# CornellHPC/HySortK

Hardware: AMD Instinct MI355X
Metric: k-mers counted/sec at K=31 (higher is better)
Workload: dtype u64

## Files before the change

hysortk_amd/csrc/hsk_parse.h:

```cpp
#pragma once
#include "hsk_device.h"

namespace hsk {

constexpr int PARSE_THREADS = 256;
constexpr int PARSE_PPT = 8;
constexpr int PARSE_TILE = PARSE_THREADS * PARSE_PPT;
constexpr int SUPERMER_CUT = 128;
constexpr int MAX_K = 95;
constexpr int HSK_MAX_TASKS = 1024;
constexpr int PARSE_WORDS = PARSE_TILE / 16 + 12;
constexpr int PARSE_HMAX = PARSE_TILE + 96;
constexpr int PARSE_RWIN = 64;
static_assert(PARSE_RWIN + PARSE_WORDS <= PARSE_THREADS, "scan_kernel prefetches the next tile with one lane per read-index entry and per word");

struct BinTable { u32 *cursor; u32 *map; u32 vmax; u32 cap_chunks; u32 *ctl; u32 *chunk_bin; ulonglong2 *items; u32 *subs; u32 *err; };

struct ParseArgs {
    const u8 *packed;
    u64 packed_bytes;
    const u64 *roff;
    const u32 *rlen;
    u64 nreads;
    int k, m;
// ... 567 lines not shown
            }
        }
        lds_barrier();
        if (a.packed_copy && tid < PARSE_TILE / 16 && bbase + 4u * (u64)tid < a.packed_bytes)
            a.packed_copy[(bbase >> 2) + tid] = __builtin_bswap32(s_words[tid]);
        {
            const u64 nb = bbase + PARSE_TILE / 4;
            pf_have = (ti + 1 < a.tiles_per_block) && (tile + 1 < tile_end) && (nb + (u64)PARSE_WORDS * 4 <= a.packed_bytes);
            if (pf_have) {
                if (tid < PARSE_RWIN) {
                    const u64 idx = s_rng[1] + tid;
                    const u64 o_ = (idx <= a.nreads) ? a.roff[idx] : RINF;
                    pf0 = (u32)o_; pf1 = (u32)(o_ >> 32);
                    pf2 = (idx < a.nreads) ? a.rlen[idx] : 0;
                } else if (tid < PARSE_RWIN + PARSE_WORDS) pf0 = reinterpret_cast<const u32 *>(a.packed + nb)[tid - PARSE_RWIN];
            }
        }
#ifdef HSK_DIAG
        if (tid == 0) { unsigned long long t_ = __builtin_amdgcn_s_memtime(); sd[1] = t_; }
#endif

        u64 h[PARSE_PPT];
        {
            const u64 w0 = bits64_be32(s_words, 16u * (u32)tid);
            const u64 rw = ~rev2(w0);
#pragma unroll
            for (int i = 0; i < PARSE_PPT; ++i) {
                const u64 fw = (w0 << (2 * i)) & mmask;
                const u64 rc = (rw << (2 * (32 - M - i))) & mmask;
                h[i] = murmur64_8(rc < fw ? rc : fw);
            }
#pragma unroll
            for (int i = 0; i < PARSE_PPT; ++i) s_hash[i * SCAN_HSTRIDE + tid] = h[i];
            if (W >= 2 * PARSE_PPT) {
                u64 bm = h[0];
#pragma unroll
                for (int i = 1; i < PARSE_PPT; ++i) bm = h[i] < bm ? h[i] : bm;
                s_bmin[tid] = bm;
            }
            for (int e = PARSE_THREADS - 1 - tid; e < W - 1; e += PARSE_THREADS) {
                const int p = PARSE_TILE + e;
                const u64 fw = bits64_be32(s_words, 2u * (u32)p) & mmask;
                const u64 tw = twin1(fw, M);
                s_hash[scan_hidx(p)] = murmur64_8(tw < fw ? tw : fw);
            }
        }
        lds_barrier();
#ifdef HSK_DIAG
        if (tid == 0) { unsigned long long t_ = __builtin_amdgcn_s_memtime(); sd[2] = t_; }
#endif

        u64 mn[PARSE_PPT];
        if (W >= PARSE_PPT) {
            u64 c = h[PARSE_PPT - 1];
            const int nfull = (W - PARSE_PPT) / PARSE_PPT;
            int j = PARSE_PPT;
            if (nfull > 0 && tid + nfull < PARSE_THREADS) {
                for (int b = 1; b <= nfull; ++b) { const u64 v = s_bmin[tid + b]; c = v < c ? v : c; }
                j = PARSE_PPT * (nfull + 1);
            }
#pragma unroll 8
            for (; j <= W - 1; ++j) { const u64 v = s_hash[scan_hidx(p0 + j)]; c = v < c ? v : c; }
            mn[PARSE_PPT - 1] = c;
            u64 suf = ~0ULL;
#pragma unroll
            for (int i = PARSE_PPT - 2; i >= 0; --i) { suf = h[i] < suf ? h[i] : suf; mn[i] = suf < c ? suf : c; }
            u64 run = ~0ULL;
#pragma unroll
            for (int i = 1; i < PARSE_PPT; ++i) { const u64 v = s_hash[scan_hidx(p0 + W + i - 1)]; run = v < run ? v : run; mn[i] = run < mn[i] ? run : mn[i]; }
        } else {
#pragma unroll
            for (int i = 0; i < PARSE_PPT; ++i) {
                u64 c = ~0ULL;
                for (int j = 0; j < W; ++j) { const u64 v = s_hash[scan_hidx(p0 + i + j)]; c = v < c ? v : c; }
                mn[i] = c;
            }
        }
        u32 vmask = 0;
        {
            const u64 g0 = gbase + p0;
            const u64 rlo = s_rng[0], rhi = s_rng[1], rb = s_rng[2];
            const bool fast = s_rng[3] != 0;
            u64 r, rstart, rend, nxt;
            if (fast) {
                u32 lo = (u32)(rlo - rb), hi = (u32)(rhi - rb);
                const u64 b0 = g0 >> 2;
                while (lo < hi) { const u32 mid = (lo + hi + 1) >> 1; if (s_roff[mid] <= b0) lo = mid; else hi = mid - 1; }
                r = rb + lo; rstart = s_roff[lo] * 4; rend = rstart + s_rlen[lo];
                nxt = (r + 1 < a.nreads) ? s_roff[lo + 1] * 4 : ~0ULL;
            } else {
                r = find_read(a.roff, rlo, rhi, g0 >> 2);
                rstart = a.roff[r] * 4; rend = rstart + a.rlen[r];
                nxt = (r + 1 < a.nreads) ? a.roff[r + 1] * 4 : ~0ULL;
            }
            if (nxt >= g0 + PARSE_PPT) {
                const long long cnt = (long long)rend - (long long)K - (long long)g0 + 1;
                vmask = cnt <= 0 ? 0u : (cnt >= PARSE_PPT ? 0xFFu : ((1u << (u32)cnt) - 1u));
            } else {
                static_assert(PARSE_PPT == 8, "two bytes of bases per lane");
                const long long cnt_lo = (long long)rend - (long long)K - (long long)g0 + 1;
                vmask = cnt_lo <= 0 ? 0u : (cnt_lo >= 4 ? 0xFu : ((1u << (u32)cnt_lo) - 1u));
                do {
                    ++r; rstart = nxt;
                    if (fast) { const u32 j = (u32)(r - rb); rend = rstart + s_rlen[j]; nxt = (r + 1 < a.nreads) ? s_roff[j + 1] * 4 : ~0ULL; }
                    else { rend = rstart + a.rlen[r]; nxt = (r + 1 < a.nreads) ? a.roff[r + 1] * 4 : ~0ULL; }
                } while (nxt <= g0 + 4);
                const long long cnt_hi = (long long)rend - (long long)K - (long long)(g0 + 4) + 1;
                vmask |= (cnt_hi <= 0 ? 0u : (cnt_hi >= 4 ? 0xFu : ((1u << (u32)cnt_hi) - 1u))) << 4;
            }
        }
        if constexpr (DROP) {
            const u32 dm = homopolymer_positions(s_words, tid, K, a.drop_mask);
            ndrop += (u32)__popc(vmask & dm);
            vmask &= ~dm;
        }
        s_last[tid] = mn[PARSE_PPT - 1];
        s_v8[tid] = (u8)vmask;
        lds_barrier();
#ifdef HSK_DIAG
        if (tid == 0) { unsigned long long t_ = __builtin_amdgcn_s_memtime(); sd[3] = t_; }
#endif

        u32 start8 = 0;
        {
            u64 pm = tid ? s_last[tid - 1] : 0;
            const u32 pv = tid ? (u32)(s_v8[tid - 1] >> 7) : 0u;
            u32 neq8 = 0;
#pragma unroll
            for (int i = 0; i < PARSE_PPT; ++i) { neq8 |= (mn[i] != pm ? 1u : 0u) << i; pm = mn[i]; }
            const u32 cut8 = ((tid & (SUPERMER_CUT / PARSE_PPT - 1)) == 0) ? 1u : 0u;
            const u32 prev8 = (vmask << 1) | pv;
            const u32 bnd8 = (~vmask | cut8 | ~prev8 | neq8) & 0xFFu;
            s_bnd8[tid] = (u8)bnd8;
            if (tid == 0) s_scan[10] = 0;
            start8 = vmask & bnd8;
        }
        u32 nrec;
        u32 off = block_excl_scan_256_lds<u32>((u32)__popc(start8), s_scan, &nrec);
#pragma unroll
        for (int i = 0; i < PARSE_PPT; ++i)
            if ((start8 >> i) & 1) { s_hash[off] = mn[i]; s_plist[off] = (u16)(p0 + i); ++off; }
        lds_barrier();
#ifdef HSK_DIAG
        if (tid == 0) { unsigned long long t_ = __builtin_amdgcn_s_memtime(); sd[4] = t_; }
#endif

        if (BINS) complete_pending(s_wprev);
        {
            const u64 *bw = reinterpret_cast<const u64 *>(s_bnd8);
            u32 *trec = a.tile_rec + tile * (u64)a.rec_cap;
            for (u32 r = tid; r < nrec; r += PARSE_THREADS) {
                const u32 p = s_plist[r];
                u32 d = fastmod64(s_hash[r], a.fm);
                const u32 sub = (u32)((s_hash[r] * 0x9E3779B97F4A7C15ULL) >> 32);
                if (a.vt_shift) d = (d << a.vt_shift) | (sub >> (32u - a.vt_shift));
                const u32 w = p >> 6;
                const u64 m = ((p & 63) == 63) ? 0ULL : (bw[w] & (~0ULL << ((p & 63) + 1)));
                u32 nb = (p | (SUPERMER_CUT - 1)) + 1;
                if (m) nb = w * 64 + (u32)__builtin_ctzll(m);
                else if ((w & 1) == 0) { const u64 m2 = bw[w + 1]; if (m2) nb = (w + 1) * 64 + (u32)__builtin_ctzll(m2); }
                u32 nk = nb - p;
                if constexpr (BINS) {
                    const BinTable &bt = *a.bins;
                    const u32 bin = xcc_nvt + d;
                    for (u32 pp = p, rest = nk, first = 1u; rest; first = 0u) {
                        const u32 piece = rest < maxk ? rest : maxk;
                        atomicAdd((unsigned long long *)&s_cur[2 * d + 0], (1ULL << 40) | (unsigned long long)piece);
                        const u32 pos = bin_reserve(bt, bin);
                        if (first && r < 2u * PARSE_THREADS) {
                            s_pend[r] = make_uint2(pp | (piece << 11) | (d << 16), sub);
                            if (r < (u32)PARSE_THREADS) { pend_pos0 = pos; pend_mask |= 1u; } else { pend_pos1 = pos; pend_mask |= 2u; }
                        } else bin_store(bt, bin_slot(bt, bin, pos, s_mc, d), bits64_be32(s_words, 2u * pp), bits64_be32(s_words, 2u * pp + 64u), piece, sub);
                        pp += piece; rest -= piece;
                    }
                    continue;
                }
                if (a.tile_sub && nk > maxk) {
                    for (u32 pp = p + maxk, rest = nk - maxk; rest; ) {
                        const u32 piece = rest < maxk ? rest : maxk;
                        const u32 rx = nrec + atomicAdd(&s_scan[10], 1u);
                        atomicAdd((unsigned long long *)&s_cur[2 * d + 0], (1ULL << 40) | (unsigned long long)piece);
                        atomicAdd((unsigned long long *)&s_cur[2 * d + 1], (unsigned long long)((piece + K - 1 + 3) >> 2));
                        if (rx < a.rec_cap) { trec[rx] = pp | ((piece - 1) << 11) | (d << 18); a.tile_sub[tile * (u64)a.rec_cap + rx] = sub; }
                        pp += piece; rest -= piece;
                    }
                    nk = maxk;
                }
                atomicAdd((unsigned long long *)&s_cur[2 * d + 0], (1ULL << 40) | (unsigned long long)nk);
                atomicAdd((unsigned long long *)&s_cur[2 * d + 1], (unsigned long long)((nk + K - 1 + 3) >> 2));
                if (r < a.rec_cap) { trec[r] = p | ((nk - 1) << 11) | (d << 18); if (a.tile_sub) a.tile_sub[tile * (u64)a.rec_cap + r] = sub; }
            }
        }
        lds_barrier();
        if (tid == 0 && !BINS) {
            const u32 nall = nrec + s_scan[10];
            a.tile_nrec[tile] = nall;
            if (nall > a.rec_cap) atomicOr(a.overflow, 1u);
        }
#ifdef HSK_DIAG
        if (tid == 0) { unsigned long long t_ = __builtin_amdgcn_s_memtime(); sd[5] = t_; }
#endif
#ifdef HSK_DIAG
        if (tid == 0) { for (int q = 0; q < 5; ++q) dacc[q] += sd[q + 1] - sd[q]; dacc[5] += 1; }
#endif
    }
#ifdef HSK_DIAG
    if (tid == 0) { for (int q = 0; q < 5; ++q) atomicAdd(&g_scan_diag[q], dacc[q]); atomicAdd(&g_scan_diag[8], dacc[5]); }
#endif
    if (BINS) complete_pending(s_words2[BINS ? (wsel ^ 1u) : 0u]);
    if constexpr (DROP) {
        u32 v = ndrop;
        for (int o = 32; o > 0; o >>= 1) v += __shfl_down(v, o, WAVE);
        if (lane_id() == 0 && v) atomicAdd(a.dropped, (unsigned long long)v);
    }
    for (u32 t = tid; t < a.ntasks; t += PARSE_THREADS) {
        u64 *o = a.blk_cnt + ((u64)blockIdx.x * a.ntasks + t) * 3;
        const u64 pk = s_cur[2 * t];
        const u64 bytes_t = BINS ? 0ULL : s_cur[2 * t + 1];
        if (a.slab == 0 || a.place_one) { o[0] = pk >> 40; o[1] = bytes_t; o[2] = pk & ((1ULL << 40) - 1); }
        else { o[0] += pk >> 40; o[1] += bytes_t; o[2] += pk & ((1ULL << 40) - 1); }
    }
}

__global__ __launch_bounds__(PARSE_THREADS) void place_kernel(ParseArgs a)
{
    if (a.place_one && a.overflow && *(const volatile u32 *)a.overflow) return;
    constexpr int RPT = PLACE_MAX_REC / PARSE_THREADS;
    __shared__ u32 s_scan[12];
    __shared__ u32 s_go[20];
    extern __shared__ __attribute__((aligned(16))) u64 s_cur[];
    const int tid = threadIdx.x;
    const int K = a.k;
    u32 *s_tcnt = reinterpret_cast<u32 *>(s_cur + a.ntasks);
    u32 *s_tpre = s_tcnt + a.ntasks;
    u32 *s_srt = s_tpre + a.ntasks;
    for (u32 t = tid; t < a.ntasks; t += PARSE_THREADS) s_cur[t] = a.blk_base[((u64)blockIdx.x * a.ntasks + t) * 2];
    const u32 G = a.place_group;
    const u32 nsl = a.nslabs > 1 ? a.nslabs : 1;
    for (u32 sl = a.place_one ? a.slab : 0; sl < (a.place_one ? a.slab + 1 : nsl); ++sl) {
    const u64 tile0 = (u64)sl * a.slab_tiles + (u64)blockIdx.x * a.tiles_per_block;
    const u64 tile_end = (nsl > 1 && ((u64)sl + 1) * a.slab_tiles < a.ntiles) ? ((u64)sl + 1) * a.slab_tiles : a.ntiles;
    for (u32 t0 = 0; t0 < a.tiles_per_block; t0 += G) {
        const u64 tfirst = tile0 + t0;
        if (tfirst >= tile_end) break;
        u32 ng = a.tiles_per_block - t0; if (ng > G) ng = G;
        if (tfirst + ng > tile_end) ng = (u32)(tile_end - tfirst);
        __syncthreads();
        if (tid == 0) {
            u32 run = 0;
            for (u32 j = 0; j < ng; ++j) { s_go[j] = run; u32 n = a.tile_nrec[tfirst + j]; run += n < a.rec_cap ? n : a.rec_cap; }
            for (u32 j = ng; j <= 16; ++j) s_go[j] = run;
        }
        for (u32 t = tid; t < a.ntasks; t += PARSE_THREADS) s_tcnt[t] = 0;
        __syncthreads();
        const u32 total = s_go[16];
        u32 rec[RPT], rnk[RPT];
#pragma unroll
        for (int x = 0; x < RPT; ++x) {
            const u32 i = x * PARSE_THREADS + tid;
            rec[x] = 0xFFFFFFFFu;
            if (i < total) {
                u32 j = 0;
                while (j + 1 < ng && s_go[j + 1] <= i) ++j;
                const u32 r = a.tile_rec[(tfirst + j) * (u64)a.rec_cap + (i - s_go[j])];
                rec[x] = r | (j << 28);
                rnk[x] = atomicAdd(&s_tcnt[(r >> 18) & 1023u], 1u);
            }
        }
        __syncthreads();
        {
            u32 c4[4], sum = 0;
#pragma unroll
            for (int j = 0; j < 4; ++j) { const u32 t = tid * 4 + j; c4[j] = t < a.ntasks ? s_tcnt[t] : 0; sum += c4[j]; }
            u32 e = block_excl_scan_256<u32>(sum, s_scan, nullptr);
#pragma unroll
            for (int j = 0; j < 4; ++j) { const u32 t = tid * 4 + j; if (t < a.ntasks) s_tpre[t] = e; e += c4[j]; }
        }
        __syncthreads();
#pragma unroll
        for (int x = 0; x < RPT; ++x)
            if (rec[x] != 0xFFFFFFFFu) s_srt[s_tpre[(rec[x] >> 18) & 1023u] + rnk[x]] = rec[x];
        __syncthreads();
        for (u32 i = tid; i < total; i += PARSE_THREADS) {
            const u32 r = s_srt[i];
            const u32 d = (r >> 18) & 1023u;
            if (a.task_skip && a.task_skip[d]) continue;
            const u64 slot = s_cur[d] + (i - s_tpre[d]);
            a.sm_len[slot] = (u8)(((r >> 11) & 127) + K);
            a.sm_gpos[slot] = (tfirst + (r >> 28)) * PARSE_TILE + (u64)(r & 2047);
        }
        __syncthreads();
        for (u32 t = tid; t < a.ntasks; t += PARSE_THREADS) s_cur[t] += s_tcnt[t];
    }
    }
}

constexpr int PLACE_ITEM_THREADS = 1024;
#ifndef PLACE_ITEM_RPT
#define PLACE_ITEM_RPT 16
#endif
constexpr u32 PLACE_ITEM_REC = PLACE_ITEM_RPT * 1024;
constexpr u32 PLACE_ITEM_TILES = PLACE_ITEM_REC / 512;
constexpr u32 PLACE_ITEM_WORDS = PLACE_ITEM_TILES * (PARSE_TILE / 16) + 8;
__global__ __launch_bounds__(PLACE_ITEM_THREADS) void place_items_kernel(ParseArgs a)
{
    if (a.place_one && a.overflow && *(const volatile u32 *)a.overflow) return;
    constexpr int RPT = PLACE_ITEM_REC / PLACE_ITEM_THREADS;
    constexpr int T = PLACE_ITEM_THREADS;
    __shared__ u32 s_w[16];
    __shared__ u32 s_go[PLACE_ITEM_TILES + 4];
    extern __shared__ __attribute__((aligned(16))) u64 s_cur[];
    const int tid = threadIdx.x;
    const u32 nt = a.ntasks;
    u32 *s_tcnt = reinterpret_cast<u32 *>(s_cur + nt);
    u32 *s_tpre = s_tcnt + nt;
    u64 *s_srt = reinterpret_cast<u64 *>(s_tpre + nt + (nt & 1u));
    u32 *s_words = reinterpret_cast<u32 *>(s_srt + PLACE_ITEM_REC);
    for (u32 t = tid; t < nt; t += T) s_cur[t] = a.blk_base[((u64)blockIdx.x * nt + t) * 2];
    const u32 G = a.place_group < PLACE_ITEM_TILES ? a.place_group : PLACE_ITEM_TILES;
    const u32 *p32 = reinterpret_cast<const u32 *>(a.packed);
    const u32 nsl = a.nslabs > 1 ? a.nslabs : 1;
    const int lane = lane_id(), wv = tid >> 6;
    for (u32 sl = a.place_one ? a.slab : 0; sl < (a.place_one ? a.slab + 1 : nsl); ++sl) {
    const u64 tile0 = (u64)sl * a.slab_tiles + (u64)blockIdx.x * a.tiles_per_block;
    const u64 tile_end = (nsl > 1 && ((u64)sl + 1) * a.slab_tiles < a.ntiles) ? ((u64)sl + 1) * a.slab_tiles : a.ntiles;
    for (u32 t0 = 0; t0 < a.tiles_per_block; t0 += G) {
        const u64 tfirst = tile0 + t0;
        if (tfirst >= tile_end) break;
        u32 ng = a.tiles_per_block - t0; if (ng > G) ng = G;
        if (tfirst + ng > tile_end) ng = (u32)(tile_end - tfirst);
        __syncthreads();
        if (tid < WAVE) {
            u32 n = 0;
            if ((u32)tid < ng) { n = a.tile_nrec[tfirst + tid]; n = n < a.rec_cap ? n : a.rec_cap; }
            const u32 inc = wave_incl_scan(n);
            if ((u32)tid < ng) s_go[tid] = inc - n;
            const u32 tot = __shfl(inc, WAVE - 1);
            if ((u32)tid >= ng && (u32)tid <= PLACE_ITEM_TILES) s_go[tid] = tot;
        }
        for (u32 t = tid; t < nt; t += T) s_tcnt[t] = 0;
        {
            const u64 w0 = tfirst * (PARSE_TILE / 16);
            const u32 nw = ng * (PARSE_TILE / 16) + 8;
            for (u32 i = tid; i < nw; i += T) {
                const u64 b = (w0 + i) * 4;
                u32 wv2 = 0;
                if (b + 4 <= a.packed_bytes) wv2 = __builtin_bswap32(p32[w0 + i]);
                else if (b < a.packed_bytes) { for (u64 q = b; q < a.packed_bytes; ++q) wv2 |= (u32)a.packed[q] << (24 - 8 * (q & 3)); }
                s_words[i] = wv2;
            }
        }
        __syncthreads();
        const u32 total = s_go[PLACE_ITEM_TILES];
        u32 rec[RPT], rnk[RPT], sub[RPT];
#pragma unroll
        for (int x = 0; x < RPT; ++x) {
            const u32 i = x * T + tid;
            rec[x] = 0xFFFFFFFFu; rnk[x] = 0; sub[x] = 0;
            if (i < total) {
                u32 lo = 0, hi = ng;
                while (hi - lo > 1) { const u32 mid = (lo + hi) >> 1; if (s_go[mid] <= i) lo = mid; else hi = mid; }
                const u64 at = (tfirst + lo) * (u64)a.rec_cap + (i - s_go[lo]);
                const u32 r = a.tile_rec[at];
                sub[x] = a.tile_sub[at];
                const u32 d = (r >> 18) & 1023u;
                rec[x] = (r & 2047u) | (((r >> 11) & 15u) << 11) | (lo << 15) | (d << 20);
                rnk[x] = atomicAdd(&s_tcnt[d], 1u);
            }
        }
        __syncthreads();
        {
            const u32 cnt = (u32)tid < nt ? s_tcnt[tid] : 0u;
            const u32 inc = wave_incl_scan(cnt);
            if (lane == WAVE - 1) s_w[wv] = inc;
            __syncthreads();
            u32 base = 0;
            for (int i = 0; i < 16; ++i) if (i < wv) base += s_w[i];
            if ((u32)tid < nt) s_tpre[tid] = base + inc - cnt;
        }
        __syncthreads();
#pragma unroll
        for (int x = 0; x < RPT; ++x)
            if (rec[x] != 0xFFFFFFFFu) s_srt[s_tpre[rec[x] >> 20] + rnk[x]] = (u64)rec[x] | ((u64)sub[x] << 32);
        __syncthreads();
        for (u32 i = tid; i < total; i += T) {
            const u64 e = s_srt[i];
            const u32 r = (u32)e;
            const u32 d = r >> 20;
            const u64 slot = s_cur[d] + (i - s_tpre[d]);
            const u32 bit0 = 2u * (((r >> 15) & 31u) * (u32)PARSE_TILE + (r & 2047u));
            const u64 w0 = bits64_be32(s_words, bit0), w1 = bits64_be32(s_words, bit0 + 64u);
            reinterpret_cast<ulonglong2 *>(a.sm_item)[slot] = make_ulonglong2(w0, (w1 & ~0xFFULL) | (u64)(((r >> 11) & 15u) + 1u));
            a.sm_sub[slot] = (u32)(e >> 32);
        }
        __syncthreads();
        for (u32 t = tid; t < nt; t += T) s_cur[t] += s_tcnt[t];
    }
    }
}

constexpr int PLACE_BYTES_THREADS = 1024;
constexpr u32 PLACE_BYTES_REC = 8192;
constexpr u32 PLACE_BYTES_TILES = 16;
constexpr u32 PLACE_BYTES_WORDS = PLACE_BYTES_TILES * (PARSE_TILE / 16) + 24;
__global__ __launch_bounds__(PLACE_BYTES_THREADS) void place_bytes_kernel(ParseArgs a)
{
    constexpr int PARSE_THREADS = PLACE_BYTES_THREADS;
    constexpr int RPT = PLACE_BYTES_REC / PARSE_THREADS;
    __shared__ u32 s_w[16];
    __shared__ u32 s_go[PLACE_BYTES_TILES + 4];
    extern __shared__ __attribute__((aligned(16))) u64 s_cur[];
    const int tid = threadIdx.x;
    const int K = a.k;
    const u32 nt = a.ntasks;
    u64 *s_curb = s_cur + nt, *s_tbase = s_curb + nt, *s_tc = s_tbase + nt;
    u32 *s_tpre = reinterpret_cast<u32 *>(s_tc + nt);
    u64 *s_srt = reinterpret_cast<u64 *>(s_tpre + 2 * nt);
    u32 *s_words = reinterpret_cast<u32 *>(s_srt + PLACE_BYTES_REC);
    unsigned short *s_sub = reinterpret_cast<unsigned short *>(s_words + PLACE_BYTES_WORDS);
    for (u32 t = tid; t < nt; t += PARSE_THREADS) {
        s_cur[t] = a.blk_base[((u64)blockIdx.x * nt + t) * 2];
        s_curb[t] = a.blk_base[((u64)blockIdx.x * nt + t) * 2 + 1];
        s_tbase[t] = a.task_base3[3 * t + 1];
    }
    const u32 G = a.place_group;
    const u32 *p32 = reinterpret_cast<const u32 *>(a.packed);
    const u32 nsl = a.nslabs > 1 ? a.nslabs : 1;
    for (u32 sl = 0; sl < nsl; ++sl) {
    const u64 tile0 = (u64)sl * a.slab_tiles + (u64)blockIdx.x * a.tiles_per_block;
    const u64 tile_end = (nsl > 1 && ((u64)sl + 1) * a.slab_tiles < a.ntiles) ? ((u64)sl + 1) * a.slab_tiles : a.ntiles;
    for (u32 t0 = 0; t0 < a.tiles_per_block; t0 += G) {
        const u64 tfirst = tile0 + t0;
        if (tfirst >= tile_end) break;
        u32 ng = a.tiles_per_block - t0; if (ng > G) ng = G;
        if (tfirst + ng > tile_end) ng = (u32)(tile_end - tfirst);
        __syncthreads();
        if (tid < WAVE) {
            u32 n = 0;
            if ((u32)tid < ng) { n = a.tile_nrec[tfirst + tid]; n = n < a.rec_cap ? n : a.rec_cap; }
            const u32 inc = wave_incl_scan(n);
            if ((u32)tid < ng) s_go[tid] = inc - n;
            const u32 tot = __shfl(inc, WAVE - 1);
            if ((u32)tid >= ng && (u32)tid <= PLACE_BYTES_TILES) s_go[tid] = tot;
        }
        for (u32 t = tid; t < nt; t += PARSE_THREADS) s_tc[t] = 0;
        {
            const u64 w0 = tfirst * (PARSE_TILE / 16);
            const u32 nw = ng * (PARSE_TILE / 16) + 24;
            for (u32 i = tid; i < nw; i += PARSE_THREADS) {
                const u64 b = (w0 + i) * 4;
                u32 wv = 0;
                if (b + 4 <= a.packed_bytes) wv = __builtin_bswap32(p32[w0 + i]);
                else if (b < a.packed_bytes) { for (u64 q = b; q < a.packed_bytes; ++q) wv |= (u32)a.packed[q] << (24 - 8 * (q & 3)); }
                s_words[i] = wv;
            }
        }
        __syncthreads();
        const u32 total = s_go[PLACE_BYTES_TILES];
        u32 rec[RPT]; u64 got[RPT]; unsigned short sb16[RPT];
#pragma unroll
        for (int x = 0; x < RPT; ++x) {
            const u32 i = x * PARSE_THREADS + tid;
            rec[x] = 0xFFFFFFFFu; got[x] = 0; sb16[x] = 0;
            if (i < total) {
                u32 j = 0, hi = ng;
                while (hi - j > 1) { const u32 mid = (j + hi) >> 1; if (s_go[mid] <= i) j = mid; else hi = mid; }
                const u32 r = a.tile_rec[(tfirst + j) * (u64)a.rec_cap + (i - s_go[j])];
                if (a.sm_sub16) sb16[x] = (unsigned short)(a.tile_sub[(tfirst + j) * (u64)a.rec_cap + (i - s_go[j])] >> 16);
                rec[x] = r | (j << 28);
                const u32 nb = (((r >> 11) & 127u) + (u32)K + 3u) >> 2;
                got[x] = atomicAdd((unsigned long long *)&s_tc[(r >> 18) & 1023u], (1ULL << 32) | (unsigned long long)nb);
            }
        }
        __syncthreads();
        {
            const u32 cnt = (u32)tid < nt ? (u32)(s_tc[tid] >> 32) : 0u;
            const u32 inc = wave_incl_scan(cnt);
            if (lane_id() == WAVE - 1) s_w[tid >> 6] = inc;
            __syncthreads();
            u32 base = 0;
            for (int i = 0; i < 16; ++i) if (i < (tid >> 6)) base += s_w[i];
            if ((u32)tid < nt) s_tpre[tid] = base + inc - cnt;
        }
        __syncthreads();
#pragma unroll
        for (int x = 0; x < RPT; ++x)
            if (rec[x] != 0xFFFFFFFFu) {
                const u32 at = s_tpre[(rec[x] >> 18) & 1023u] + (u32)(got[x] >> 32);
                s_srt[at] = (u64)rec[x] | (got[x] << 32);
                if (a.sm_sub16) s_sub[at] = sb16[x];
            }
        __syncthreads();
        for (u32 i = tid; i < total; i += PARSE_THREADS) {
            const u64 e = s_srt[i];
            const u32 r = (u32)e, bo = (u32)(e >> 32);
            const u32 d = (r >> 18) & 1023u;
            if (a.task_skip && a.task_skip[d]) continue;
            const u64 slot = s_cur[d] + (i - s_tpre[d]);
            const u64 babs = s_curb[d] + bo;
            const u32 len = ((r >> 11) & 127u) + (u32)K;
            const u32 nb = (len + 3) >> 2;
            a.sm_len[slot] = (u8)len;
            if (a.sm_boff) a.sm_boff[slot] = (u32)(babs - s_tbase[d]);
            if (a.sm_sub16) a.sm_sub16[slot] = s_sub[i];
            if (a.sm_gpos) a.sm_gpos[slot] = (tfirst + (r >> 28)) * PARSE_TILE + (u64)(r & 2047);
            const u32 bit0 = 2u * ((r >> 28) * (u32)PARSE_TILE + (r & 2047u));
            const u64 tailmask = (len & 3u) ? ~(u64)(0xFFu >> (2 * (len & 3u))) : ~0ULL;
            u8 *dst = a.sm_bytes + babs;
            if (nb >= 8) {
                const u32 nfull = nb >> 3, rem = nb & 7u;
                for (u32 q = 0; q < nfull; ++q) {
                    u64 v = bits64_be32(s_words, bit0 + 64u * q);
                    if (rem == 0 && q + 1 == nfull) v &= tailmask;
                    *reinterpret_cast<u64 *>(dst + 8u * q) = __builtin_bswap64(v);
                }
                if (rem) { const u64 v = bits64_be32(s_words, bit0 + 8u * (nb - 8u)) & tailmask; *reinterpret_cast<u64 *>(dst + (nb - 8u)) = __builtin_bswap64(v); }
            } else {
                const u64 v = bits64_be32(s_words, bit0) & (tailmask << (8u * (8u - nb)) | ~(~0ULL >> (8u * (nb - 1u))));
                for (u32 q = 0; q < nb; ++q) dst[q] = (u8)(v >> (56u - 8u * q));
            }
        }
        __syncthreads();
        for (u32 t = tid; t < nt; t += PARSE_THREADS) { const u64 c = s_tc[t]; s_cur[t] += c >> 32; s_curb[t] += c & 0xFFFFFFFFu; }
    }
    }
}

__device__ __forceinline__ u64 s_gpos_load(const u64 *p, u64 i) { return p[i]; }
__global__ void resolve_pos_rid_kernel(const u64 *sm_gpos, u64 n, const u64 *roff, u64 nreads, int64_t rid_base, u32 *sm_pos, int32_t *sm_rid,
                                       const u32 *tile_r0, u64 ntiles)
{
    const u64 stride = (u64)gridDim.x * blockDim.x;
    for (u64 s = (u64)blockIdx.x * blockDim.x + threadIdx.x; s < n; s += stride) {
        const u64 g = s_gpos_load(sm_gpos, s);
        u64 lo = 0, hi = nreads - 1;
        if (tile_r0) {
            const u64 tile = g / PARSE_TILE;
            lo = tile_r0[tile];
            hi = (tile + 1 < ntiles) ? tile_r0[tile + 1] : nreads - 1;
            if (hi < lo) hi = lo;
        }
        const u64 r = find_read(roff, lo, hi, g >> 2);
        sm_pos[s] = (u32)(g - roff[r] * 4);
        sm_rid[s] = (int32_t)(rid_base + (int64_t)r);
    }
}

__global__ void prefix_reads_kernel(const u64 *roff, u64 nreads, u64 bytes, u64 *out)
{
    if (threadIdx.x || blockIdx.x) return;
    const u64 r = nreads ? find_read(roff, 0, nreads - 1, bytes) : 0;
    out[0] = r; out[1] = nreads ? roff[r] : 0;
}

__global__ void index_check_kernel(const u64 *roff, const u32 *rlen, u64 nreads, u64 packed_bytes, u32 *err)
{
    const u64 stride = (u64)gridDim.x * blockDim.x;
    bool bad = false;
    for (u64 r = (u64)blockIdx.x * blockDim.x + threadIdx.x; r < nreads; r += stride) {
        const u64 o = roff[r], end = o + ((u64)rlen[r] + 3) / 4;
        if (end > packed_bytes || end < o) bad = true;
        if (r == 0 ? o != 0 : o < roff[r - 1] + ((u64)rlen[r - 1] + 3) / 4) bad = true;
    }
    if (bad) atomicOr(err, 32u);
}

__global__ void rlen_fill_kernel(u32 *rlen, u64 nreads, u32 len)
{
    const u64 stride = (u64)gridDim.x * blockDim.x;
    for (u64 r = (u64)blockIdx.x * blockDim.x + threadIdx.x; r < nreads; r += stride) rlen[r] = len;
}

constexpr int ROFF_TILE = PARSE_THREADS * 8;
__global__ __launch_bounds__(PARSE_THREADS) void roff_tilesum_kernel(const u32 *rlen, u64 nreads, u64 *tile_sum)
{
    __shared__ u64 s_scr[8];
    const u64 base = (u64)blockIdx.x * ROFF_TILE + (u64)threadIdx.x * 8;
    u64 sum = 0;
#pragma unroll
    for (int i = 0; i < 8; ++i) if (base + i < nreads) sum += ((u64)rlen[base + i] + 3) >> 2;
    u64 tot;
    (void)block_excl_scan_256<u64>(sum, s_scr, &tot);
    if (threadIdx.x == 0) tile_sum[blockIdx.x] = tot;
}
__global__ __launch_bounds__(PARSE_THREADS) void roff_tilescan_kernel(u64 *tile_sum, u64 ntiles)
{
    __shared__ u64 s_scr[8];
    __shared__ u64 s_carry;
    if (threadIdx.x == 0) s_carry = 0;
    __syncthreads();
    for (u64 base = 0; base < ntiles; base += (u64)PARSE_THREADS * 8) {
        const u64 t0 = base + (u64)threadIdx.x * 8;
        u64 v[8], sum = 0;
#pragma unroll
        for (int i = 0; i < 8; ++i) { v[i] = t0 + i < ntiles ? tile_sum[t0 + i] : 0; sum += v[i]; }
        u64 tot;
        u64 ex = block_excl_scan_256<u64>(sum, s_scr, &tot) + s_carry;
#pragma unroll
        for (int i = 0; i < 8; ++i) { if (t0 + i < ntiles) tile_sum[t0 + i] = ex; ex += v[i]; }
        __syncthreads();
        if (threadIdx.x == 0) s_carry += tot;
        __syncthreads();
    }
}
__global__ __launch_bounds__(PARSE_THREADS) void roff_write_kernel(const u32 *rlen, u64 nreads, const u64 *tile_off, u64 *roff)
{
    __shared__ u64 s_scr[8];
    const u64 base = (u64)blockIdx.x * ROFF_TILE + (u64)threadIdx.x * 8;
    u64 nb[8], sum = 0;
#pragma unroll
    for (int i = 0; i < 8; ++i) { nb[i] = base + i < nreads ? ((u64)rlen[base + i] + 3) >> 2 : 0; sum += nb[i]; }
    u64 ex = block_excl_scan_256<u64>(sum, s_scr, nullptr) + tile_off[blockIdx.x];
#pragma unroll
    for (int i = 0; i < 8; ++i) { if (base + i < nreads) roff[base + i] = ex; ex += nb[i]; }
}
__device__ __forceinline__ void col_sums(const u64 *blk_cnt, u32 nblocks, u32 ntasks, u32 t, u64 &s, u64 &b, u64 &k)
{
    constexpr int U = 8;
    u32 blk = 0;
    for (; blk + U <= nblocks; blk += U) {
        u64 v[U][3];
#pragma unroll
        for (int u = 0; u < U; ++u) { const u64 *c = blk_cnt + ((u64)(blk + u) * ntasks + t) * 3; v[u][0] = c[0]; v[u][1] = c[1]; v[u][2] = c[2]; }
#pragma unroll
        for (int u = 0; u < U; ++u) { s += v[u][0]; b += v[u][1]; k += v[u][2]; }
    }
    for (; blk < nblocks; ++blk) { const u64 *c = blk_cnt + ((u64)blk * ntasks + t) * 3; s += c[0]; b += c[1]; k += c[2]; }
}

__global__ void task_totals_kernel(const u64 *blk_cnt, u32 nblocks, u32 ntasks, u64 *task_tot)
{
    const u32 t = threadIdx.x;
    if (t >= ntasks) return;
    u64 s = 0, b = 0, k = 0;
    col_sums(blk_cnt, nblocks, ntasks, t, s, b, k);
    task_tot[3 * t] = s; task_tot[3 * t + 1] = b; task_tot[3 * t + 2] = k;
}

__global__ void parse_scan_kernel(const u64 *blk_cnt, u32 nblocks, u32 ntasks, const u32 *order, const u8 *skip,
                                  u64 *task_tot, u64 *task_base, u64 *blk_base, u64 *run = nullptr)
{
    __shared__ u64 s_tot[HSK_MAX_TASKS * 3];
    const u32 t = threadIdx.x;
    const bool live = t < ntasks && !(skip && skip[t]);
    if (t < ntasks) {
        u64 s = 0, b = 0, k = 0;
        if (live) col_sums(blk_cnt, nblocks, ntasks, t, s, b, k);
        s_tot[3 * t] = s; s_tot[3 * t + 1] = b; s_tot[3 * t + 2] = k;
        task_tot[3 * t] = s; task_tot[3 * t + 1] = b; task_tot[3 * t + 2] = k;
    }
    __syncthreads();
    {
        __shared__ u64 s_part[3][16];
        const u32 task = t < ntasks ? order[t] : 0u;
        u64 v0 = t < ntasks ? s_tot[3 * task] : 0, v1 = t < ntasks ? s_tot[3 * task + 1] : 0, v2 = t < ntasks ? s_tot[3 * task + 2] : 0;
        const int lane = lane_id(), w = (int)(t >> 6);
        const u64 i0 = wave_incl_scan(v0), i1 = wave_incl_scan(v1), i2 = wave_incl_scan(v2);
        if (lane == WAVE - 1) { s_part[0][w] = i0; s_part[1][w] = i1; s_part[2][w] = i2; }
        __syncthreads();
        u64 b0 = run ? run[0] : 0, b1 = run ? run[1] : 0, b2 = run ? run[2] : 0, t0 = 0, t1 = 0, t2 = 0;
        for (int i = 0; i < 16; ++i) {
            const u64 p0 = s_part[0][i], p1 = s_part[1][i], p2 = s_part[2][i];
            if (i < w) { b0 += p0; b1 += p1; b2 += p2; }
            t0 += p0; t1 += p1; t2 += p2;
        }
        if (t < ntasks) { task_base[3 * task] = b0 + i0 - v0; task_base[3 * task + 1] = b1 + i1 - v1; task_base[3 * task + 2] = b2 + i2 - v2; }
        __syncthreads();
        if (t == 0 && run) { run[0] += t0; run[1] += t1; run[2] += t2; }
    }
    __syncthreads();
    if (t < ntasks) {
        u64 s = task_base[3 * t], b = task_base[3 * t + 1];
        constexpr int U = 16;
        u32 blk = 0;
        for (; blk + U <= nblocks; blk += U) {
            u64 v[U][2];
#pragma unroll
            for (int u = 0; u < U; ++u) { const u64 *c = blk_cnt + ((u64)(blk + u) * ntasks + t) * 3; v[u][0] = c[0]; v[u][1] = c[1]; }
#pragma unroll
            for (int u = 0; u < U; ++u) {
                u64 *o = blk_base + ((u64)(blk + u) * ntasks + t) * 2;
                o[0] = s; o[1] = b;
                if (live) { s += v[u][0]; b += v[u][1]; }
            }
        }
        for (; blk < nblocks; ++blk) {
            const u64 *c = blk_cnt + ((u64)blk * ntasks + t) * 3;
            u64 *o = blk_base + ((u64)blk * ntasks + t) * 2;
            o[0] = s; o[1] = b;
            if (live) { s += c[0]; b += c[1]; }
        }
    }
}

constexpr u32 PS_SEGS = 16;
constexpr u32 PS_THREADS = 256;
__global__ __launch_bounds__(PS_THREADS) void parse_scan_part_kernel(const u64 *blk_cnt, u32 nblocks, u32 ntasks, const u8 *skip, u64 *part)
{
    const u32 t = blockIdx.x * PS_THREADS + threadIdx.x, seg = blockIdx.y;
    if (t >= ntasks) return;
// ... 67 lines not shown
```

Baseline: 80.94 billion.

## Software-pipeline place_items_kernel by prefetching next step's records and packed words

```diff
diff --git a/hysortk_amd/csrc/hsk_parse.h b/hysortk_amd/csrc/hsk_parse.h
--- a/hysortk_amd/csrc/hsk_parse.h
+++ b/hysortk_amd/csrc/hsk_parse.h
@@ -893,11 +893,15 @@
 constexpr u32 PLACE_ITEM_REC = PLACE_ITEM_RPT * 1024;
 constexpr u32 PLACE_ITEM_TILES = PLACE_ITEM_REC / 512;
 constexpr u32 PLACE_ITEM_WORDS = PLACE_ITEM_TILES * (PARSE_TILE / 16) + 8;
+struct PlaceItemStep { u32 sl, t0, ng; u64 tfirst; bool ok; };
 __global__ __launch_bounds__(PLACE_ITEM_THREADS) void place_items_kernel(ParseArgs a)
 {
     if (a.place_one && a.overflow && *(const volatile u32 *)a.overflow) return;
     constexpr int RPT = PLACE_ITEM_REC / PLACE_ITEM_THREADS;
     constexpr int T = PLACE_ITEM_THREADS;
+    constexpr int WPT = (PLACE_ITEM_WORDS + T - 1) / T;
+    constexpr int LPR = (RPT + 5) / 6;
+    static_assert(PLACE_ITEM_TILES <= 32, "a record's tile of the step takes 5 bits");
     __shared__ u32 s_w[16];
     __shared__ u32 s_go[PLACE_ITEM_TILES + 4];
     extern __shared__ __attribute__((aligned(16))) u64 s_cur[];
@@ -911,49 +915,93 @@
     const u32 G = a.place_group < PLACE_ITEM_TILES ? a.place_group : PLACE_ITEM_TILES;
     const u32 *p32 = reinterpret_cast<const u32 *>(a.packed);
     const u32 nsl = a.nslabs > 1 ? a.nslabs : 1;
+    const u32 sl_end = a.place_one ? a.slab + 1 : nsl;
     const int lane = lane_id(), wv = tid >> 6;
-    for (u32 sl = a.place_one ? a.slab : 0; sl < (a.place_one ? a.slab + 1 : nsl); ++sl) {
-    const u64 tile0 = (u64)sl * a.slab_tiles + (u64)blockIdx.x * a.tiles_per_block;
-    const u64 tile_end = (nsl > 1 && ((u64)sl + 1) * a.slab_tiles < a.ntiles) ? ((u64)sl + 1) * a.slab_tiles : a.ntiles;
-    for (u32 t0 = 0; t0 < a.tiles_per_block; t0 += G) {
-        const u64 tfirst = tile0 + t0;
-        if (tfirst >= tile_end) break;
-        u32 ng = a.tiles_per_block - t0; if (ng > G) ng = G;
-        if (tfirst + ng > tile_end) ng = (u32)(tile_end - tfirst);
-        __syncthreads();
+    auto step_at = [&](u32 sl, u32 t0) {
+        PlaceItemStep s = {0, 0, 0, 0, false};
+        for (; sl < sl_end; ++sl, t0 = 0) {
+            if (t0 >= a.tiles_per_block) continue;
+            const u64 tile_end = (nsl > 1 && ((u64)sl + 1) * a.slab_tiles < a.ntiles) ? ((u64)sl + 1) * a.slab_tiles : a.ntiles;
+            const u64 tfirst = (u64)sl * a.slab_tiles + (u64)blockIdx.x * a.tiles_per_block + t0;
+            if (tfirst >= tile_end) continue;
+            u32 ng = a.tiles_per_block - t0; if (ng > G) ng = G;
+            if (tfirst + ng > tile_end) ng = (u32)(tile_end - tfirst);
+            s.sl = sl; s.t0 = t0; s.ng = ng; s.tfirst = tfirst; s.ok = true;
+            break;
+        }
+        return s;
+    };
+    auto load_nrec = [&](const PlaceItemStep &s) {
+        u32 n = 0;
+        if (tid < WAVE && s.ok && (u32)tid < s.ng) { n = a.tile_nrec[s.tfirst + tid]; n = n < a.rec_cap ? n : a.rec_cap; }
+        return n;
+    };
+    auto write_go = [&](const PlaceItemStep &s, u32 n) {
         if (tid < WAVE) {
-            u32 n = 0;
-            if ((u32)tid < ng) { n = a.tile_nrec[tfirst + tid]; n = n < a.rec_cap ? n : a.rec_cap; }
             const u32 inc = wave_incl_scan(n);
-            if ((u32)tid < ng) s_go[tid] = inc - n;
+            if ((u32)tid < s.ng) s_go[tid] = inc - n;
             const u32 tot = __shfl(inc, WAVE - 1);
-            if ((u32)tid >= ng && (u32)tid <= PLACE_ITEM_TILES) s_go[tid] = tot;
-        }
-        for (u32 t = tid; t < nt; t += T) s_tcnt[t] = 0;
-        {
-            const u64 w0 = tfirst * (PARSE_TILE / 16);
-            const u32 nw = ng * (PARSE_TILE / 16) + 8;
-            for (u32 i = tid; i < nw; i += T) {
-                const u64 b = (w0 + i) * 4;
-                u32 wv2 = 0;
-                if (b + 4 <= a.packed_bytes) wv2 = __builtin_bswap32(p32[w0 + i]);
-                else if (b < a.packed_bytes) { for (u64 q = b; q < a.packed_bytes; ++q) wv2 |= (u32)a.packed[q] << (24 - 8 * (q & 3)); }
-                s_words[i] = wv2;
-            }
-        }
-        __syncthreads();
-        const u32 total = s_go[PLACE_ITEM_TILES];
-        u32 rec[RPT], rnk[RPT], sub[RPT];
+            if ((u32)tid >= s.ng && (u32)tid <= PLACE_ITEM_TILES) s_go[tid] = tot;
+        }
+    };
+    u32 rec[RPT], rnk[RPT], sub[RPT], lop[LPR], words[WPT];
+    auto fetch = [&](const PlaceItemStep &s, u32 total) {
+#pragma unroll
+        for (int q = 0; q < LPR; ++q) lop[q] = 0;
 #pragma unroll
         for (int x = 0; x < RPT; ++x) {
             const u32 i = x * T + tid;
-            rec[x] = 0xFFFFFFFFu; rnk[x] = 0; sub[x] = 0;
+            rec[x] = 0; sub[x] = 0;
             if (i < total) {
-                u32 lo = 0, hi = ng;
+                u32 lo = 0, hi = s.ng;
                 while (hi - lo > 1) { const u32 mid = (lo + hi) >> 1; if (s_go[mid] <= i) lo = mid; else hi = mid; }
-                const u64 at = (tfirst + lo) * (u64)a.rec_cap + (i - s_go[lo]);
-                const u32 r = a.tile_rec[at];
+                const u64 at = (s.tfirst + lo) * (u64)a.rec_cap + (i - s_go[lo]);
+                rec[x] = a.tile_rec[at];
                 sub[x] = a.tile_sub[at];
+                lop[x / 6] |= lo << (5 * (x % 6));
+            }
+        }
+        const u64 w0 = s.tfirst * (PARSE_TILE / 16);
+        const u32 nw = s.ng * (PARSE_TILE / 16) + 8;
+#pragma unroll
+        for (int q = 0; q < WPT; ++q) {
+            const u32 i = q * T + tid;
+            words[q] = 0;
+            if (i < nw) {
+                const u64 b = (w0 + i) * 4;
+                if (b + 4 <= a.packed_bytes) words[q] = p32[w0 + i];
+                else if (b < a.packed_bytes) {
+                    u32 wv2 = 0;
+                    for (u64 q2 = b; q2 < a.packed_bytes; ++q2) wv2 |= (u32)a.packed[q2] << (24 - 8 * (q2 & 3));
+                    words[q] = __builtin_bswap32(wv2);
+                }
+            }
+        }
+    };
+    auto put_words = [&](const PlaceItemStep &s) {
+        const u32 nw = s.ng * (PARSE_TILE / 16) + 8;
+#pragma unroll
+        for (int q = 0; q < WPT; ++q) { const u32 i = q * T + tid; if (i < nw) s_words[i] = __builtin_bswap32(words[q]); }
+    };
+    PlaceItemStep cur = step_at(a.place_one ? a.slab : 0, 0);
+    if (!cur.ok) return;
+    write_go(cur, load_nrec(cur));
+    for (u32 t = tid; t < nt; t += T) s_tcnt[t] = 0;
+    __syncthreads();
+    u32 total = s_go[PLACE_ITEM_TILES];
+    fetch(cur, total);
+    put_words(cur);
+    __syncthreads();
+    for (;;) {
+        const PlaceItemStep nxt = step_at(cur.sl, cur.t0 + G);
+        const u32 nrec_nxt = load_nrec(nxt);
+#pragma unroll
+        for (int x = 0; x < RPT; ++x) {
+            const u32 i = x * T + tid;
+            const u32 r = rec[x];
+            rec[x] = 0xFFFFFFFFu; rnk[x] = 0;
+            if (i < total) {
+                const u32 lo = (lop[x / 6] >> (5 * (x % 6))) & 31u;
                 const u32 d = (r >> 18) & 1023u;
                 rec[x] = (r & 2047u) | (((r >> 11) & 15u) << 11) | (lo << 15) | (d << 20);
                 rnk[x] = atomicAdd(&s_tcnt[d], 1u);
@@ -969,11 +1017,14 @@
             for (int i = 0; i < 16; ++i) if (i < wv) base += s_w[i];
             if ((u32)tid < nt) s_tpre[tid] = base + inc - cnt;
         }
+        if (nxt.ok) write_go(nxt, nrec_nxt);
         __syncthreads();
 #pragma unroll
         for (int x = 0; x < RPT; ++x)
             if (rec[x] != 0xFFFFFFFFu) s_srt[s_tpre[rec[x] >> 20] + rnk[x]] = (u64)rec[x] | ((u64)sub[x] << 32);
         __syncthreads();
+        u32 total_nxt = 0;
+        if (nxt.ok) { total_nxt = s_go[PLACE_ITEM_TILES]; fetch(nxt, total_nxt); }
         for (u32 i = tid; i < total; i += T) {
             const u64 e = s_srt[i];
             const u32 r = (u32)e;
@@ -985,8 +1036,11 @@
             a.sm_sub[slot] = (u32)(e >> 32);
         }
         __syncthreads();
-        for (u32 t = tid; t < nt; t += T) s_cur[t] += s_tcnt[t];
-    }
+        for (u32 t = tid; t < nt; t += T) { s_cur[t] += s_tcnt[t]; s_tcnt[t] = 0; }
+        if (!nxt.ok) break;
+        put_words(nxt);
+        __syncthreads();
+        cur = nxt; total = total_nxt;
     }
 }
 
```

New measurement: 83.26 billion (median of 6 runs). 1.03x the previous value.
